# mhozza/covest

Hardware: NVIDIA B200
Metric: loglik_point_bin_evals_per_sec (higher is better)
Workload: dtype f64

## Files before the change

### covest_b200/csrc/capi.cu

```cuda
#include <cuda_runtime.h>

#include <cmath>
#include <cstdio>
#include <cstdlib>
#include <algorithm>
#include <cstring>
#include <string>
#include <utility>
#include <vector>

#include "../../include/covest_b200.h"
#include "cvtables.h"
#include "factored.h"
#include "faithful.h"
#include "kernels.h"
#include "kmers.h"

#define CVB_CHUNK_POINTS (1LL << 22)
#define CVB_MAX_TIMED_CHUNKS 64
#define CVB_TOPK_RADIX_MIN 32768

struct cvb_ctx {
    int device = 0;
    int n_sm = 0;
// ... 277 lines not shown
            const char *rows = getenv("COVEST_B200_ROWS");
            const bool compact = !(rows && !strcmp(rows, "full"));
            CvHostTables RT;
            const bool row_tables = compact && tail == 0.0 && cv_build_row_tables(T, bin_j, bin_h, RT);
            c->fdesc = m;
            if (row_tables) {
                CvModelDesc &f = c->fdesc;
                f.n_groups = RT.n_groups;
                f.na = RT.na;
                f.n_blocks = RT.n_blocks;
                f.tab.slot_mult = f.tab.slot_h = nullptr;
                f.tab.slot_bin = nullptr;
                if ((e = upload_profile_tables(c, RT, f.tab)) != cudaSuccess) break;
            }
            const CvHostTables &FT = row_tables ? RT : T;
            std::vector<int> line_map;
            std::vector<double2> mh;
            std::vector<double> row_h;
            cvf_build_slots(FT.slot_mult, FT.slot_h, compact, row_tables, line_map, mh, row_h, &c->slots.sum_line);
            c->slots.nsteps = (int)(row_h.size() / 64);
            if ((e = upload(c, line_map, &c->slots.line_map)) != cudaSuccess) break;
            if ((e = upload(c, mh, &c->slots.slot_mh)) != cudaSuccess) break;
            if ((e = upload(c, cvf_step_masks(row_h), &c->slots.step_mask)) != cudaSuccess) break;
            c->slots.counts_first = cvf_counts_first(row_h);
            std::vector<double> lt(2 * CV_LOG_N);
            cv_log_table(lt.data());
            if ((e = upload(c, lt, &c->d_log_tab)) != cudaSuccess) break;
        }
        if (const char *pm = getenv("COVEST_B200_PATH"))
            c->path_mode = !strcmp(pm, "direct") ? 1 : !strcmp(pm, "factored") ? 2 : !strcmp(pm, "gemm") ? 3
                           : !strcmp(pm, "prefix") ? 4 : !strcmp(pm, "faithful") ? 5 : 0;
        if (const char *wl = getenv("COVEST_B200_PROFILE_MIB"))
            if (atoll(wl) > 0)
                c->w_limit = (size_t)atoll(wl) * (1 << 20) / sizeof(double);
        if (const char *po = getenv("COVEST_B200_POISON")) {
            c->poison = !strcmp(po, "nan") ? 0xFF : !strcmp(po, "finite") ? 0x7F : 0;
            if (!c->poison && *po) {
                rc = fail(nullptr, CVB_EINVAL, "COVEST_B200_POISON must be nan or finite");
                break;
// ... 645 lines not shown

extern "C" int cvb_last_path_info(cvb_ctx *ctx, double *out, int n_out)
{
    if (!ctx || !out || n_out < 1)
        return CVB_EINVAL;
    CU(cudaSetDevice(ctx->device), "cudaSetDevice");
    double v[CVB_PATH_INFO_LEN] = {0};
    v[0] = ctx->last_path;
    {
        unsigned long long fixed = 0;
        CU(cudaMemcpy(&fixed, ctx->d_fixed, sizeof(fixed), cudaMemcpyDeviceToHost), "cudaMemcpy");
        v[9] = (double)fixed;
    }
    if (ctx->last_path >= 2) {
        v[10] = (double)ctx->fw.analytic;
        v[11] = (double)(ctx->slots.nsteps * 64 - (ctx->slots.sum_line >= 0 ? 32 : 0));
        const CvFactorWork &w = ctx->fw;
        v[1] = (double)w.n_groups;
        v[2] = (double)w.n_tiles;
        v[3] = (double)w.n_items;
        v[4] = (double)w.w_doubles;
        v[8] = (double)w.n_runs;
        if (w.timed && w.ev[0]) {
            float ms = 0.f;
            CU(cudaEventSynchronize(w.ev[3]), "cudaEventSynchronize");
            CU(cudaEventElapsedTime(&ms, w.ev[0], w.ev[1]), "cudaEventElapsedTime");
            v[5] = ms;
            CU(cudaEventElapsedTime(&ms, w.ev[1], w.ev[2]), "cudaEventElapsedTime");
            v[6] = ms;
            CU(cudaEventElapsedTime(&ms, w.ev[2], w.ev[3]), "cudaEventElapsedTime");
            v[7] = ms;
// ... 330 lines not shown
```

### covest_b200/csrc/factored.cu

```cuda
#include "factored.h"

#include <cub/device/device_radix_sort.cuh>
#include <cub/block/block_scan.cuh>
#include <cub/device/device_scan.cuh>

#include <algorithm>
#include <cstring>
#include <vector>

#include "kdevice.h"

#define CVF_M 128
#define CVF_NS 64
#define CVF_KC 16
#define CVF_THREADS 256
#define CVF_OBITS 20
#define CVF_TILE_DOUBLES (CVF_KC * CVF_NS)

struct CvfPlan {
    unsigned long long *keys, *keys_alt;
    unsigned int *idx, *idx_alt;
    const unsigned int *idx_sorted;
    int *othr;
    int *head, *gid;
// ... 319 lines not shown
{
    int lo = 0, hi = n;
    while (hi - lo > 1) {
        const int step = (hi - lo + 31) >> 5;
        const int p = lo + (lane + 1) * step;
        const bool ok = p < hi && __ldg(start + p) <= x;
        const int cnt = __popc(__ballot_sync(CV_FULL_MASK, ok));
        const int nlo = lo + cnt * step;
        hi = min(nlo + step, hi);
        lo = nlo;
    }
    return lo;
}

#define CVF_STAGE_DOUBLES (CV_GB * CV_NA_MAX * CV_W)

template <int NA>
__device__ __forceinline__ void cvf_store_profile(int lane, int blk, int o, int nsteps,
                                                  const double *__restrict__ slot_mult ,
                                                  const int *__restrict__ line_map, int sum_line, bool sums,
                                                  double *__restrict__ Wg, double *stage, const double *acc)
{
    const int r = lane >> 2, q = lane & 3;
#pragma unroll
    for (int mt = 0; mt < NA; mt++)
#pragma unroll
        for (int c = 0; c < 2; c++) {
            const int chunk = (2 * q + c) ^ (r & 1);
            *reinterpret_cast<double2 *>(stage + (NA * r + mt) * CV_W + 2 * chunk) =
                make_double2(acc[4 * mt + c], acc[4 * mt + 2 + c]);
        }
    __syncwarp();
    double *row0 = Wg + (long long)(o - 1) * nsteps * CVF_NS + lane * 2;
    double2 rest = make_double2(0.0, 0.0);
#pragma unroll
    for (int ns = 0; ns < 2 * NA; ns++) {
        const int row = 4 * ns + (lane >> 3);
        const int chunk = (lane & 7) ^ ((row / NA) & 1);
        double2 v = *reinterpret_cast<const double2 *>(stage + row * CV_W + 2 * chunk);
        const double2 mm = __ldg(reinterpret_cast<const double2 *>(slot_mult) + (blk * (2 * NA) + ns) * 32 + lane);
        v.x = cv_mul(v.x, mm.x);
        v.y = cv_mul(v.y, mm.y);
        const int line = __ldg(line_map + blk * (2 * NA) + ns);
        if (line >= 0) {
            *reinterpret_cast<double2 *>(row0 + line * CVF_NS) = v;
        } else if (sums) {
            rest.x = cv_add(rest.x, v.x);
            rest.y = cv_add(rest.y, v.y);
        }
    }
    if (sum_line >= 0) {
        double *dst = Wg + ((long long)(o - 1) * nsteps + sum_line) * CVF_NS + lane;
        double sum = 0.0;
        if (sums) {
            sum = cv_add(rest.x, rest.y);
            if (blk > 0)
                sum = cv_add(*dst, sum);
        }
        dst[0] = sum;
        dst[32] = 0.0;
    }
    __syncwarp();
}

template <int NA>
__device__ __forceinline__ void cvf_profile_item(int lane, const CvModelDesc &m, CvWarpMem &M,
                                                 int o0, int omax4, int nsteps, const int *__restrict__ line_map,
                                                 int sum_line, double *__restrict__ Wg, double *stage)
{
    const int sp = cvf_copy_slots(m.n_err);
    const int cpt = cvf_copies_per_tile(m.n_err);
    const int kpc = sp >> 2;
    const bool sums = m.tail != 0.0;
    for (int oa = o0; oa < o0 + CVF_KC && oa <= omax4; oa += cpt) {
        cv_w_mass(lane, m, oa, cpt * sp, sp, M);
        __syncwarp();
        const CvTerm tm = cv_w_term(lane, m, oa, cpt * sp, sp, 0, 1.0, M);
        for (int blk = 0; blk < m.n_blocks; blk++) {
            const CvLaneGroup G = cv_lane_group(lane, m, blk, M);
            cv_w_prep<NA>(lane, m, blk, tm, M);
            __syncwarp();
            for (int cc = 0; cc < cpt; cc++) {
                double acc[4 * NA];
#pragma unroll
                for (int i = 0; i < 4 * NA; i++)
                    acc[i] = 0.0;
                cv_w_fused<NA>(lane, G, cc * kpc, (cc + 1) * kpc, *M.fx, acc);
                cvf_store_profile<NA>(lane, blk, oa + cc, nsteps, m.tab.slot_mult_pair, line_map, sum_line, sums, Wg, stage,
                                      acc);
            }
            __syncwarp();
        }
    }
}

__global__ void __launch_bounds__(32 * CV_WARPS_MAX, 1)
cvf_profile_kernel(const __grid_constant__ CvModelDesc m, const __grid_constant__ CvLattice lat,
                   const double *__restrict__ params, int clip, CvfPlan pl, int n_groups,
                   int first_item, int n_items, double *__restrict__ W, long long w_base, int nsteps,
                   const int *__restrict__ line_map, int sum_line, unsigned long long *counter, int groups_staged)
{
    extern __shared__ __align__(16) unsigned char cv_smem_raw[];
    const int lane = threadIdx.x & 31, warp = threadIdx.x >> 5;
    const int S = m.n_err;
    CvWarpMem M;
    {
        double *tab = reinterpret_cast<double *>(cv_smem_raw);
        const int ntab = groups_staged * CV_GD;
        unsigned char *wbase = cv_smem_raw + (size_t)ntab * sizeof(double) + (size_t)warp * cv_warp_bytes(S);
        CvWarpFixed *fx = reinterpret_cast<CvWarpFixed *>(wbase);
        cv_warp_mem_carve(M, fx, reinterpret_cast<double *>(wbase + sizeof(CvWarpFixed)), S);
        for (int i = threadIdx.x; i < ntab; i += blockDim.x)
            tab[i] = m.tab.grp[i];
        M.grp = tab;
    }
// ... 10 lines not shown
            break;
        const int item = first_item + (int)it;
        const int g = cvf_find_warp(pl.item_start, n_groups, item, lane);
        const int kchunk = item - pl.item_start[g];
        const int a = pl.g_start[g];
        const int omax = pl.g_omax[g] - 1;
        const int omax4 = (omax + 3) & ~3;
        double row[CV_MAX_PARAMS];
        cvf_raw_row(m, lat, params, pl.idx_sorted[a], row);
        __syncwarp();
        cv_w_header(lane, m, row, clip, M);
        __syncwarp();
        double *Wg = W + (pl.w_off[g] - w_base);
        const int o0 = kchunk * CVF_KC + 1;
        switch (m.na) {
        case 1: cvf_profile_item<1>(lane, m, M, o0, omax4, nsteps, line_map, sum_line, Wg, stage); break;
        case 2: cvf_profile_item<2>(lane, m, M, o0, omax4, nsteps, line_map, sum_line, Wg, stage); break;
        case 4: cvf_profile_item<4>(lane, m, M, o0, omax4, nsteps, line_map, sum_line, Wg, stage); break;
        default: cvf_profile_item<8>(lane, m, M, o0, omax4, nsteps, line_map, sum_line, Wg, stage); break;
        }
    }
}

#define CVF_STAGES 4
struct CvfSmem {
    double2 Bs[CVF_STAGES][CVF_TILE_DOUBLES / 2];
    double2 As[CVF_STAGES][CVF_M * CVF_KC / 2];
    double red_sum[2][CVF_M];
    double red_mh[2][CVF_M], red_ml[2][CVF_M];
    double log_tab[2 * CV_LOG_N];
    int othr[CVF_M];
    unsigned int pidx[CVF_M];
    int tile;
};
// ... 448 lines not shown

__device__ __forceinline__ int cvf_count_below(const int *a, int n, int x, bool or_equal)
{
    int lo = 0, hi = n;
    while (lo < hi) {
        const int mid = (lo + hi) >> 1;
        const int v = a[mid];
        if (v < x || (or_equal && v == x))
            lo = mid + 1;
        else
            hi = mid;
    }
    return lo;
}

template <bool MASS, bool FULL, bool ONE, int NW, int SL>
__global__ void __launch_bounds__(32 * NW, CVF_WARPS_SM / NW)
cvf_prefix_kernel(const __grid_constant__ CvModelDesc m, const __grid_constant__ CvLattice lat,
                  const double *__restrict__ params, int clip, CvfPlan pl, int first_tile, int n_tiles,
                  const double *__restrict__ W, long long w_base, const double2 *__restrict__ slot_mh,
                  const double *__restrict__ log_tab, int nsteps, int nslots, double *__restrict__ out_ll,
                  unsigned long long *counter, double *__restrict__ scratch)
{
    constexpr int PT_ = 32 * NW, PW_ = NW;
    constexpr int PASS_ = PT_ * SL;
    constexpr int RING_ = CVF_PD * SL * PT_ * 8;
    constexpr int TBUF_ = PW_ * CVF_PE * CVF_PEW;
    extern __shared__ __align__(16) unsigned char cvf_smem_raw[];
    CvfPrefixSmem &S = *reinterpret_cast<CvfPrefixSmem *>(cvf_smem_raw);
    const int tid = threadIdx.x, lane = tid & 31, warp = tid >> 5;
    double *ring = reinterpret_cast<double *>(cvf_smem_raw + CVF_SMEM_HEAD) + tid;
    double *tbuf = reinterpret_cast<double *>(cvf_smem_raw + CVF_SMEM_HEAD + RING_) +
// ... 87 lines not shown
                S.ev[rank] = e;
            }
            if (tid < 2) {
                CvfEvent e;
                e.q1 = e.two = e.many = 0.0;
                e.info = e.need = 0;
                S.ev[npts + tid] = e;
            }
            __syncthreads();

            for (int pass0 = 0; pass0 < nslots; pass0 += PASS_) {
                const int u0 = (pass0 >> 5) + warp;
                const double *src0 = Wg + u0 * 32 + lane;
                constexpr long long SRC_STEP = (long long)PW_ * 32;
                double hcnt[SL];
                int log_mask = 0;
                bool live[SL];
#pragma unroll
                for (int i = 0; i < SL; i++) {
                    const int u = u0 + i * PW_;
                    live[i] = FULL || u * 32 < nslots;
                    const int e = (u & 1) * 32 + lane, L = e >> 1;
                    const int slot = (u >> 1) * CVF_NS + 16 * (L >> 3) + (L & 7) + 8 * (e & 1);
                    hcnt[i] = live[i] ? __ldg(&slot_mh[slot].y) : 0.0;
                    log_mask |= (__any_sync(CV_FULL_MASK, hcnt[i] != 0.0) ? 1 : 0) << i;
                }
                const bool wide = !ONE && log_mask == (1 << SL) - 1;
                auto pair_fast = [&](const double *pa, const double *pb) {
                    unsigned int worst = 0;
#pragma unroll
                    for (int i = 0; i < SL; i++) {
                        const unsigned int ca = (unsigned int)(__double2hiint(pa[i]) - CVF_FAST_LO),
                                           cb = (unsigned int)(__double2hiint(pb[i]) - CVF_FAST_LO);
                        if (hcnt[i] != 0.0)
                            worst = max(worst, max(ca, cb));
                    }
                    return worst < CVF_FAST_SPAN;
                };
                int o_req = 1;
                unsigned int dst_req = ring_s;
                const double *src_req = src0;
                const double *src_far = src0 + (long long)CVF_PL2 * row_stride;
// ... 176 lines not shown
                            const double2 qt = cvf_lds128(ev_a);
                            q1 = qt.x;
                            two = qt.y;
                            cvf_lds_event(ev_a, many, info, need);
                        }
                        k++;
                        double ma = 0.0, mb = 0.0, mla = 0.0, mlb = 0.0;
                        if (MASS) {
#pragma unroll
                            for (int i = 0; i < SL; i++) {
                                cvf_two_sum_acc(ma, mla, pa[i]);
                                cvf_two_sum_acc(mb, mlb, pb[i]);
                            }
                        }
                        double sa = 0.0, sb = 0.0;
                        if (ONE ? log_mask != 0 : log_mask == 1) {
                            const unsigned int ca = (unsigned int)(__double2hiint(pa[0]) - CVF_FAST_LO),
                                               cb = (unsigned int)(__double2hiint(pb[0]) - CVF_FAST_LO);
                            double la, lb;
                            if (ca < CVF_FAST_SPAN && cb < CVF_FAST_SPAN) {
                                la = cvf_log_fast(pa[0], log_s);
                                lb = cvf_log_fast(pb[0], log_s);
                            } else {
                                la = cvf_safe_log(pa[0], log_s);
                                lb = cvf_safe_log(pb[0], log_s);
                            }
                            sa = cv_mul(hcnt[0], la);
                            sb = cv_mul(hcnt[0], lb);
                            if (hcnt[0] == 0.0)
                                sa = sb = 0.0;
                        } else if (wide && pair_fast(pa, pb)) {
#pragma unroll
                            for (int i = 0; i < SL; i++) {
                                const double la = cvf_log_fast(pa[i], log_s),
                                             lb = cvf_log_fast(pb[i], log_s);
                                double ta = cv_mul(hcnt[i], la), tb = cv_mul(hcnt[i], lb);
                                if (hcnt[i] == 0.0)
                                    ta = tb = 0.0;
                                sa = cv_add(sa, ta);
                                sb = cv_add(sb, tb);
                            }
                        } else if (!ONE && log_mask) {
#pragma unroll
                            for (int i = 0; i < SL; i++)
                                if ((log_mask >> i) & 1) {
                                    const unsigned int ca = (unsigned int)(__double2hiint(pa[i]) - CVF_FAST_LO),
                                                       cb = (unsigned int)(__double2hiint(pb[i]) - CVF_FAST_LO);
                                    double la, lb;
                                    if (ca < CVF_FAST_SPAN && cb < CVF_FAST_SPAN) {
                                        la = cvf_log_fast(pa[i], log_s);
                                        lb = cvf_log_fast(pb[i], log_s);
                                    } else {
                                        la = cvf_safe_log(pa[i], log_s);
                                        lb = cvf_safe_log(pb[i], log_s);
                                    }
                                    double ta = cv_mul(hcnt[i], la), tb = cv_mul(hcnt[i], lb);
                                    if (hcnt[i] == 0.0)
                                        ta = tb = 0.0;
                                    sa = cv_add(sa, ta);
                                    sb = cv_add(sb, tb);
                                }
                        }
                        if (pending == CVF_PE - 1) {
                            flush();
                            tb_a = tbuf_s;
                        }
                        cvf_sts64(tb_a, sa);
                        cvf_sts64(tb_a + CVF_PEW * 8, sb);
                        if (MASS) {
                            cvf_sts64(tb_a + TBUF_ * 8, ma);
                            cvf_sts64(tb_a + CVF_PEW * 8 + TBUF_ * 8, mb);
                            cvf_sts64(tb_a + 2 * TBUF_ * 8, mla);
                            cvf_sts64(tb_a + CVF_PEW * 8 + 2 * TBUF_ * 8, mlb);
                        }
                        tb_a += 2 * CVF_PEW * 8;
                        if (lane == pending)
// ... 22 lines not shown
                        CVF_CASE(2)
                        CVF_CASE(3)
#undef CVF_CASE
                    }
                    q1 = qt_next.x;
                    two = qt_next.y;
                    many = many_next;
                    info = info_next;
                    need = need_next;
                    double sum = 0.0, mh = 0.0, ml = 0.0;
                    if (MASS) {
#pragma unroll
                        for (int i = 0; i < SL; i++)
                            cvf_two_sum_acc(mh, ml, p[i]);
                    }
                    if (ONE ? log_mask != 0 : log_mask == 1) {
                        double term = cv_mul(hcnt[0], cvf_safe_log(p[0], log_s));
                        if (hcnt[0] == 0.0)
                            term = 0.0;
                        sum = term;
                    } else if (!ONE && log_mask) {
#pragma unroll
                        for (int i = 0; i < SL; i++)
                            if ((log_mask >> i) & 1) {
                                double term = cv_mul(hcnt[i], cvf_safe_log(p[i], log_s));
                                if (hcnt[i] == 0.0)
                                    term = 0.0;
                                sum = cv_add(sum, term);
                            }
                    }
                    cvf_sts64(tb_a, sum);
                    if (MASS) {
                        cvf_sts64(tb_a + TBUF_ * 8, mh);
                        cvf_sts64(tb_a + 2 * TBUF_ * 8, ml);
                    }
                    tb_a += CVF_PEW * 8;
                    if (lane == pending)
                        mypt = pt;
                    if (++pending == CVF_PE) {
                        flush();
                        tb_a = tbuf_s;
                    }
                }
                if (pending)
// ... 453 lines not shown
    double *A = wk.W + w_need;
    if (wk.poison) {
        CVF_CK(cudaMemsetAsync(wk.W, wk.poison, (w_need + a_need) * sizeof(double), stream));
        CVF_CK(cudaMemsetAsync(wk.d_scratch, wk.poison, (size_t)n_sm * 32 * 3 * CVF_PB * sizeof(double), stream));
    }

    const size_t wb = cv_warp_bytes(m.n_err);
    const int groups_staged = m.n_blocks * CV_GB;
    const size_t tab = (size_t)groups_staged * CV_GD * sizeof(double);
    const size_t wb1 = wb + CVF_STAGE_DOUBLES * sizeof(double);
    int k1_warps = (int)std::min<long long>(CV_WARPS_MAX, ((long long)smem_max - (long long)tab) / (long long)wb1);
    if (k1_warps < 1)
        return cudaErrorInvalidConfiguration;
    const size_t k1_smem = tab + (size_t)k1_warps * wb1;
    const bool want_mass = m.tail != 0.0;
    const int kp_slots = slots_padded - (sl.sum_line >= 0 ? (want_mass || nsteps == 1 ? 32 : CVF_NS) : 0);
    const int kp_half = kp_slots / 32;
    int kp_nw = 8, kp_sl = 4;
    if (kp_half <= 24) {
        static const int nws[] = {1, 2, 3, 4, 6, 8};
        int n3 = 8, n4 = 8;
        for (int i = 5; i >= 0; i--) {
            if (nws[i] * 3 >= kp_half && nws[i] != 4 && nws[i] != 8)
                n3 = nws[i];
            if (nws[i] * 4 >= kp_half)
                n4 = nws[i];
        }
        if (n3 <= n4) {
            kp_nw = n3;
            kp_sl = 3;
        } else {
            kp_nw = n4;
        }
    }
    const size_t kp_smem = cvf_prefix_smem_bytes(want_mass, kp_nw, kp_sl);
    const bool full_passes = kp_slots % (8 * 32 * 4) == 0;
    const bool counts_first = sl.counts_first;
    typedef decltype(&cvf_prefix_kernel<true, true, true, 8, 4>) CvfPrefixFn;
    CvfPrefixFn kp = nullptr;
    const bool full_one = kp_slots == kp_nw * 32 * kp_sl;
#define CVF_PICK(nw_, sl_)                                                                                          \
    (full_one ? (want_mass ? cvf_prefix_kernel<true, true, false, nw_, sl_> : cvf_prefix_kernel<false, true, false, nw_, sl_>) \
              : (want_mass ? cvf_prefix_kernel<true, false, false, nw_, sl_> : cvf_prefix_kernel<false, false, false, nw_, sl_>))
    switch (kp_nw * 10 + kp_sl) {
    case 13: kp = CVF_PICK(1, 3); break;
    case 14: kp = CVF_PICK(1, 4); break;
    case 23: kp = CVF_PICK(2, 3); break;
    case 24: kp = CVF_PICK(2, 4); break;
    case 33: kp = CVF_PICK(3, 3); break;
    case 34: kp = CVF_PICK(3, 4); break;
    case 44: kp = CVF_PICK(4, 4); break;
    case 63: kp = CVF_PICK(6, 3); break;
    case 64: kp = CVF_PICK(6, 4); break;
    default:
        kp = want_mass ? (full_passes ? (counts_first ? cvf_prefix_kernel<true, true, true, 8, 4> : cvf_prefix_kernel<true, true, false, 8, 4>)
                                      : (counts_first ? cvf_prefix_kernel<true, false, true, 8, 4> : cvf_prefix_kernel<true, false, false, 8, 4>))
                       : (full_passes ? (counts_first ? cvf_prefix_kernel<false, true, true, 8, 4> : cvf_prefix_kernel<false, true, false, 8, 4>)
                                      : (counts_first ? cvf_prefix_kernel<false, false, true, 8, 4> : cvf_prefix_kernel<false, false, false, 8, 4>));
    }
#undef CVF_PICK
    CVF_CK(cudaFuncSetAttribute(cvf_profile_kernel, cudaFuncAttributeMaxDynamicSharedMemorySize, (int)k1_smem));
    CVF_CK(cudaFuncSetAttribute(cvf_gemm_kernel, cudaFuncAttributeMaxDynamicSharedMemorySize,
                                (int)sizeof(CvfSmem)));
    CVF_CK(cudaFuncSetAttribute(kp, cudaFuncAttributeMaxDynamicSharedMemorySize, (int)kp_smem));
    if (wk.timed)
        CVF_CK(cudaEventRecord(wk.ev[1], stream));
    for (size_t i = 0; i + 1 < cut.size(); i++) {
        const int g0 = cut[i], g1 = cut[i + 1];
        const int item0 = ranged ? h_item[g0] : 0, item1 = ranged ? h_item[g1] : (int)n_items;
        const int tile0 = ranged ? h_tile[g0] : 0, tile1 = ranged ? h_tile[g1] : (int)n_tiles;
        const long long w0 = ranged ? h_woff[g0] : 0;
        const long long a0 = ranged ? h_achunk[g0] : 0;
        CVF_CK(cudaMemsetAsync(wk.d_counters, 0, 2 * sizeof(unsigned long long), stream));
        if (item1 > item0) {
            const int items = item1 - item0;
            int grid = (items + k1_warps - 1) / k1_warps;
            if (grid > n_sm)
                grid = n_sm;
            cvf_profile_kernel<<<grid, 32 * k1_warps, k1_smem, stream>>>(
                m, lat, params, clip, pl, (int)n_groups, item0, items, wk.W, w0, nsteps, sl.line_map, sl.sum_line,
                wk.d_counters, groups_staged);
            CVF_CK(cudaGetLastError());
            wk.launches++;
        }
        if (tile1 > tile0) {
            const int tiles = tile1 - tile0;
            if (!prefix) {
                cvf_weights_kernel<<<tiles, CVF_THREADS, 0, stream>>>(m, lat, params, clip, pl, tile0, tiles, A, a0);
                CVF_CK(cudaGetLastError());
                wk.launches++;
            }
            if (analytic) {
                cvf_lattice_order<<<(unsigned int)((tiles + tb - 1) / tb), tb, 0, stream>>>(
                    TD, g0, g1, (int)(n_tiles / n_groups), pl.t_order_alt + tile0);
                CVF_CK(cudaGetLastError());
                pl.t_sorted = pl.t_order_alt + tile0;
            } else {
                cub::DoubleBuffer<int> dk(pl.t_key + tile0, pl.t_key_alt + tile0);
                cub::DoubleBuffer<int> dv(pl.t_order + tile0, pl.t_order_alt + tile0);
                size_t tb_ = tmp_bytes;
                CVF_CK(cub::DeviceRadixSort::SortPairsDescending(tmp, tb_, dk, dv, tiles, 0, 32, stream));
                pl.t_sorted = dv.Current();
            }
            if (wk.timed && i + 2 == cut.size())
                CVF_CK(cudaEventRecord(wk.ev[2], stream));
            int grid = tiles < 2 * n_sm ? tiles : 2 * n_sm;
            if (prefix) {
                const int per_sm = std::max(1, std::min(CVF_WARPS_SM / kp_nw, (int)((size_t)smem_max / (kp_smem + 1024))));
                grid = tiles < per_sm * n_sm ? tiles : per_sm * n_sm;
                kp<<<grid, 32 * kp_nw, kp_smem, stream>>>(m, lat, params, clip, pl, tile0, tiles, wk.W, w0, slot_mh,
                                                           log_tab, nsteps, kp_slots, out_ll, wk.d_counters + 1,
                                                           wk.d_scratch);
            } else {
                cvf_gemm_kernel<<<grid, CVF_THREADS, sizeof(CvfSmem), stream>>>(
                    m, pl, tile0, tiles, wk.W, w0, A, a0, slot_mh, step_mask, log_tab, nsteps, out_ll,
                    wk.d_counters + 1);
            }
            CVF_CK(cudaGetLastError());
            wk.launches += 2;
        }
    }
    if (wk.timed)
        CVF_CK(cudaEventRecord(wk.ev[3], stream));
// ... 4 lines not shown
```

### covest_b200/csrc/factored.h

```cpp
#pragma once
#include <cuda_runtime.h>
#include <stdint.h>

#include <vector>

#include "kernels.h"

struct CvfLatticeCache {
    std::vector<double> key;
    std::vector<int> host;
    int M = 0, R = 0, nq = 0, nT = 0, omax = 0;
    int *dev = nullptr;
    size_t dev_cap = 0;
    int *pinned = nullptr;
    size_t pinned_cap = 0;
    cudaEvent_t uploaded = nullptr;
};

struct CvFactorWork {
    void *plan = nullptr;
    size_t plan_cap = 0;
    double *W = nullptr;
    size_t w_cap = 0;
    long long *h_header = nullptr;
// ... 1 lines not shown
    unsigned long long *d_counters = nullptr;
    double *d_scratch = nullptr;
    cudaEvent_t ev[4] = {nullptr, nullptr, nullptr, nullptr};
    bool timed = false;
    long long n_groups = 0, n_tiles = 0, n_items = 0, w_doubles = 0, n_runs = 0;
    int prefix = 0;
    int launches = 0;
    int analytic = 0;
    int poison = 0;
    CvfLatticeCache lattice;
    double gemm_fma = 0.0;
};

struct CvfSlots {
    int nsteps = 0;
    int sum_line = -1;
    const int *line_map = nullptr;
    const double2 *slot_mh = nullptr;
    const int *step_mask = nullptr;
    bool counts_first = false;
};

static inline void cvf_build_slots(const std::vector<double> &slot_mult, const std::vector<double> &slot_h,
                                   bool compact, bool sums, std::vector<int> &line_map, std::vector<double2> &mh,
                                   std::vector<double> &row_h, int *sum_line)
{
    const size_t lines = slot_h.size() / 64;
    line_map.assign(lines, -1);
    mh.clear();
    row_h.clear();
    int kept = 0;
    for (size_t l = 0; l < lines; l++) {
        bool counts = !compact;
        for (int i = 0; i < 64 && !counts; i++)
            counts = slot_h[l * 64 + i] != 0.0;
        if (!counts)
            continue;
        line_map[l] = kept++;
        for (int i = 0; i < 64; i++) {
            double2 v;
            v.x = slot_mult[l * 64 + i];
            v.y = slot_h[l * 64 + i];
            mh.push_back(v);
            row_h.push_back(v.y);
        }
    }
    *sum_line = -1;
    if ((size_t)kept < lines || sums) {
        *sum_line = kept;
        for (int i = 0; i < 64; i++) {
            double2 v;
            v.x = 1.0;
            v.y = 0.0;
            mh.push_back(v);
            row_h.push_back(0.0);
        }
    }
}

bool cvf_supported(const CvModelDesc &m);

cudaError_t cvf_eval(const CvModelDesc &m, const CvLattice &lat, const double *const *lat_axes_host,
                     const double *params, long long n,
                     int clip, double *out_ll, const CvfSlots &sl,
                     const double *log_tab, CvFactorWork &wk, int n_sm, int smem_max, size_t w_limit,
                     double min_group, double min_run, int kernel_mode, cudaStream_t stream,
                     int *used);

static inline std::vector<int> cvf_step_masks(const std::vector<double> &slot_h)
{
    std::vector<int> out(slot_h.size() / 32, 0);
    for (size_t s = 0; s < slot_h.size(); s++)
        if (slot_h[s] != 0.0) {
            const int in32 = (int)(s & 31), nt = in32 >> 3, c = in32 & 1;
            out[s / 32] |= 1 << (2 * nt + c);
        }
    return out;
}

static inline bool cvf_counts_first(const std::vector<double> &slot_h)
{
    for (size_t s = 0; s < slot_h.size(); s++)
        if (slot_h[s] != 0.0 && (((2 * (s / 64) + (s % 64) / 32) % 32) >> 3) != 0)
            return false;
    return true;
}

void cvf_release(CvFactorWork &wk);
```

### covest_b200/engine.py

```python
import ctypes
import math
import os

import numpy as np

from . import _capi


class DeviceError(RuntimeError):
    """An error reported by libcovest_b200 (bad argument or CUDA failure)."""


def default_device():
    for var in ('COVEST_B200_DEVICE', 'LOCAL_RANK'):
        v = os.environ.get(var)
        if v not in (None, ''):
            return int(v)
    return 0


def _is_torch_cuda(x):
    return hasattr(x, 'data_ptr') and hasattr(x, 'is_cuda') and x.is_cuda


# ... 216 lines not shown
                    'cvb_last_kernel_ms')
        return ms.value, n.value

    def last_launches(self):
        n = ctypes.c_int()
        self._check(self._lib.cvb_last_kernel_ms(self._ctx, None, ctypes.byref(n)), 'cvb_last_kernel_ms')
        return n.value

    PATH_AUTO, PATH_PER_POINT, PATH_FACTORED, PATH_FACTORED_GEMM, PATH_FACTORED_PREFIX = 0, 1, 2, 3, 4
    PATH_TERM_BY_TERM = 5

    def set_path(self, mode):
        self._check(self._lib.cvb_set_path(self._ctx, int(mode)), 'cvb_set_path')

    def last_path_info(self):
        buf = (ctypes.c_double * 12)()
        self._check(self._lib.cvb_last_path_info(self._ctx, buf, 12), 'cvb_last_path_info')
        v = list(buf)
        return {'path': {1: 'per-point', 2: 'factored', 3: 'factored', 4: 'term-by-term'}.get(int(v[0]), 'none'),
                'kernel': {1: 'cv_loglik_kernel', 2: 'cvf_gemm_kernel', 3: 'cvf_prefix_kernel',
                           4: 'cv_faithful_kernel'}.get(int(v[0]), 'none'),
                'groups': int(v[1]), 'tiles': int(v[2]), 'items': int(v[3]), 'profile_doubles': int(v[4]),
                'plan_ms': v[5], 'profile_ms': v[6], 'gemm_ms': v[7], 'q_runs': int(v[8]),
                'refined_points': int(v[9]), 'analytic_plan': bool(v[10]), 'row_slots': int(v[11])}

    @property
    def sm_count(self):
        return self._lib.cvb_device_sm_count(self._ctx)
```

### include/covest_b200.h

```cpp
#ifndef COVEST_B200_H
#define COVEST_B200_H

#include <stdint.h>

#ifdef __cplusplus
extern "C" {
#endif

#if defined(__GNUC__)
#define CVB_API __attribute__((visibility("default")))
#else
#define CVB_API
#endif

#define CVB_OK 0
#define CVB_EINVAL (-1)
#define CVB_ECUDA (-2)
#define CVB_ENOMEM (-3)

#define CVB_MODEL_BASIC 0
#define CVB_MODEL_REPEATS 1

typedef struct cvb_ctx cvb_ctx;

// ... 23 lines not shown
CVB_API int cvb_lattice_eval(cvb_ctx *ctx, const int32_t *axis_len, const double *axis_values,
                     int64_t first, int64_t stride, int64_t block, int64_t count, double *out_ll,
                     int k_best, double *out_rows, void *stream);

CVB_API int cvb_lattice_profile(cvb_ctx *ctx, const int32_t *axis_len, const double *axis_values,
                                int64_t first, int64_t stride, int64_t block, int64_t count,
                                uint32_t keep_mask, double *out_rows, void *stream);

CVB_API int cvb_fp64_peak(cvb_ctx *ctx, int kind, int reps, double *out_tflops);

CVB_API int cvb_set_timing(cvb_ctx *ctx, int enabled);
CVB_API int cvb_last_kernel_ms(cvb_ctx *ctx, double *out_ms, int *out_launches);

CVB_API int cvb_set_path(cvb_ctx *ctx, int mode);

#define CVB_PATH_INFO_LEN 12
CVB_API int cvb_last_path_info(cvb_ctx *ctx, double *out, int n_out);

CVB_API int cvb_n_param(const cvb_ctx *ctx);
CVB_API int cvb_device_sm_count(const cvb_ctx *ctx);
CVB_API const char *cvb_version(void);

typedef struct cvb_kmer_table cvb_kmer_table;

CVB_API int cvb_kmer_table_create(int k, int64_t capacity, int part, int n_parts, int device,
                                  cvb_kmer_table **out);
CVB_API void cvb_kmer_table_destroy(cvb_kmer_table *t);
CVB_API const char *cvb_kmer_last_error(const cvb_kmer_table *t);

CVB_API int cvb_kmer_clear(cvb_kmer_table *t, void *stream);

// ... 14 lines not shown
```

Baseline: 774.6 billion.

## Pack nonzero-count profile slots densely instead of keeping whole 64-slot lines

The profile layout now keeps only the individual slots with nonzero histogram weight, packed contiguously with a per-slot gather map into the swizzled staging buffer, rather than keeping whole 64-slot lines. The prefix kernel therefore reads and takes logs over fewer profile entries, and the log_mask / counts_first special-case branches are dropped in favour of a uniform loop. The profile store becomes an indexed gather with partial stores. SL>4 variants get a lower occupancy bound. The risks are gather overhead and unaligned scalar stores in the profile kernel.

```diff
diff --git a/covest_b200/csrc/capi.cu b/covest_b200/csrc/capi.cu
--- a/covest_b200/csrc/capi.cu
+++ b/covest_b200/csrc/capi.cu
@@ -315,15 +315,18 @@
                 if ((e = upload_profile_tables(c, RT, f.tab)) != cudaSuccess) break;
             }
             const CvHostTables &FT = row_tables ? RT : T;
-            std::vector<int> line_map;
-            std::vector<double2> mh;
-            std::vector<double> row_h;
-            cvf_build_slots(FT.slot_mult, FT.slot_h, compact, row_tables, line_map, mh, row_h, &c->slots.sum_line);
-            c->slots.nsteps = (int)(row_h.size() / 64);
-            if ((e = upload(c, line_map, &c->slots.line_map)) != cudaSuccess) break;
-            if ((e = upload(c, mh, &c->slots.slot_mh)) != cudaSuccess) break;
-            if ((e = upload(c, cvf_step_masks(row_h), &c->slots.step_mask)) != cudaSuccess) break;
-            c->slots.counts_first = cvf_counts_first(row_h);
+            CvfRowLayout L;
+            cvf_build_slots(FT.slot_mult, FT.slot_h, FT.n_blocks, compact, row_tables, L);
+            c->slots.nsteps = L.nsteps;
+            c->slots.body = L.body;
+            c->slots.sum_half = L.sum_half;
+            c->slots.line_slots = L.line_slots;
+            if ((e = upload(c, L.at, &c->slots.at)) != cudaSuccess) break;
+            if ((e = upload(c, L.mult, &c->slots.mult)) != cudaSuccess) break;
+            if ((e = upload(c, L.blk_first, &c->slots.blk_first)) != cudaSuccess) break;
+            if ((e = upload(c, L.in_row, &c->slots.in_row)) != cudaSuccess) break;
+            if ((e = upload(c, L.mh, &c->slots.slot_mh)) != cudaSuccess) break;
+            if ((e = upload(c, cvf_step_masks(L.row_h), &c->slots.step_mask)) != cudaSuccess) break;
             std::vector<double> lt(2 * CV_LOG_N);
             cv_log_table(lt.data());
             if ((e = upload(c, lt, &c->d_log_tab)) != cudaSuccess) break;
@@ -999,7 +1002,8 @@
     }
     if (ctx->last_path >= 2) {
         v[10] = (double)ctx->fw.analytic;
-        v[11] = (double)(ctx->slots.nsteps * 64 - (ctx->slots.sum_line >= 0 ? 32 : 0));
+        v[11] = (double)ctx->slots.line_slots;
+        v[12] = (double)(ctx->slots.sum_half >= 0 ? 32 * (ctx->slots.sum_half + 1) : 64 * ctx->slots.nsteps);
         const CvFactorWork &w = ctx->fw;
         v[1] = (double)w.n_groups;
         v[2] = (double)w.n_tiles;
diff --git a/covest_b200/csrc/factored.cu b/covest_b200/csrc/factored.cu
--- a/covest_b200/csrc/factored.cu
+++ b/covest_b200/csrc/factored.cu
@@ -357,11 +357,11 @@
 }
 
 #define CVF_STAGE_DOUBLES (CV_GB * CV_NA_MAX * CV_W)
+#define CVF_GATHER 4
 
 template <int NA>
-__device__ __forceinline__ void cvf_store_profile(int lane, int blk, int o, int nsteps,
-                                                  const double *__restrict__ slot_mult ,
-                                                  const int *__restrict__ line_map, int sum_line, bool sums,
+__device__ __forceinline__ void cvf_store_profile(int lane, int blk, int k0, int k1, int o, const CvfSlots &sl,
+                                                  const double *__restrict__ slot_mult , bool sums,
                                                   double *__restrict__ Wg, double *stage, const double *acc)
 {
     const int r = lane >> 2, q = lane & 3;
@@ -369,31 +369,66 @@
     for (int mt = 0; mt < NA; mt++)
 #pragma unroll
         for (int c = 0; c < 2; c++) {
-            const int chunk = (2 * q + c) ^ (r & 1);
+            const int chunk = (2 * q + c) ^ cvf_stage_swizzle(NA * r + mt, NA);
             *reinterpret_cast<double2 *>(stage + (NA * r + mt) * CV_W + 2 * chunk) =
                 make_double2(acc[4 * mt + c], acc[4 * mt + 2 + c]);
         }
     __syncwarp();
-    double *row0 = Wg + (long long)(o - 1) * nsteps * CVF_NS + lane * 2;
+    double *row = Wg + (long long)(o - 1) * sl.nsteps * CVF_NS;
+    const int ka = 16 * (lane >> 3) + (lane & 7);
+    for (int l0 = k0 >> 6; 64 * l0 < k1; l0 += CVF_GATHER) {
+        int2 at[CVF_GATHER];
+        double2 mm[CVF_GATHER];
+#pragma unroll
+        for (int i = 0; i < CVF_GATHER; i++) {
+            const int a = 64 * (l0 + i) + ka, b = a + 8;
+            const bool ia = a >= k0 && a < k1, ib = b >= k0 && b < k1;
+            at[i] = make_int2(-2, -2);
+            mm[i] = make_double2(0.0, 0.0);
+            if (ia || ib) {
+                at[i] = __ldg(sl.at + 32 * (l0 + i) + lane);
+                mm[i] = __ldg(sl.mult + 32 * (l0 + i) + lane);
+                at[i].x = ia ? at[i].x : -2;
+                at[i].y = ib ? at[i].y : -2;
+            }
+        }
+#pragma unroll
+        for (int i = 0; i < CVF_GATHER; i++) {
+            double2 v = make_double2(0.0, 0.0);
+            if (at[i].x >= 0)
+                v.x = cv_mul(stage[at[i].x], mm[i].x);
+            if (at[i].y >= 0)
+                v.y = cv_mul(stage[at[i].y], mm[i].y);
+            double *dst = row + 64 * (l0 + i) + 2 * lane;
+            if (at[i].x >= -1 && at[i].y >= -1) {
+                *reinterpret_cast<double2 *>(dst) = v;
+            } else {
+                if (at[i].x >= -1)
+                    dst[0] = v.x;
+                if (at[i].y >= -1)
+                    dst[1] = v.y;
+            }
+        }
+    }
     double2 rest = make_double2(0.0, 0.0);
-#pragma unroll
-    for (int ns = 0; ns < 2 * NA; ns++) {
-        const int row = 4 * ns + (lane >> 3);
-        const int chunk = (lane & 7) ^ ((row / NA) & 1);
-        double2 v = *reinterpret_cast<const double2 *>(stage + row * CV_W + 2 * chunk);
-        const double2 mm = __ldg(reinterpret_cast<const double2 *>(slot_mult) + (blk * (2 * NA) + ns) * 32 + lane);
-        v.x = cv_mul(v.x, mm.x);
-        v.y = cv_mul(v.y, mm.y);
-        const int line = __ldg(line_map + blk * (2 * NA) + ns);
-        if (line >= 0) {
-            *reinterpret_cast<double2 *>(row0 + line * CVF_NS) = v;
-        } else if (sums) {
-            rest.x = cv_add(rest.x, v.x);
-            rest.y = cv_add(rest.y, v.y);
-        }
-    }
-    if (sum_line >= 0) {
-        double *dst = Wg + ((long long)(o - 1) * nsteps + sum_line) * CVF_NS + lane;
+    if (sums) {
+#pragma unroll
+        for (int ns = 0; ns < 2 * NA; ns++) {
+            const int srow = 4 * ns + (lane >> 3);
+            const int chunk = (lane & 7) ^ cvf_stage_swizzle(srow, NA);
+            double2 v = *reinterpret_cast<const double2 *>(stage + srow * CV_W + 2 * chunk);
+            const double2 mm = __ldg(reinterpret_cast<const double2 *>(slot_mult) + (blk * (2 * NA) + ns) * 32 + lane);
+            v.x = cv_mul(v.x, mm.x);
+            v.y = cv_mul(v.y, mm.y);
+            const unsigned long long in_row = __ldg(sl.in_row + blk * (2 * NA) + ns) >> (16 * (lane >> 3) + (lane & 7));
+            if (!(in_row & 1))
+                rest.x = cv_add(rest.x, v.x);
+            if (!((in_row >> 8) & 1))
+                rest.y = cv_add(rest.y, v.y);
+        }
+    }
+    if (sl.sum_half >= 0) {
+        double *dst = row + 32 * sl.sum_half + lane;
         double sum = 0.0;
         if (sums) {
             sum = cv_add(rest.x, rest.y);
@@ -401,15 +436,16 @@
                 sum = cv_add(*dst, sum);
         }
         dst[0] = sum;
-        dst[32] = 0.0;
+        if (!(sl.sum_half & 1))
+            dst[32] = 0.0;
     }
     __syncwarp();
 }
 
 template <int NA>
 __device__ __forceinline__ void cvf_profile_item(int lane, const CvModelDesc &m, CvWarpMem &M,
-                                                 int o0, int omax4, int nsteps, const int *__restrict__ line_map,
-                                                 int sum_line, double *__restrict__ Wg, double *stage)
+                                                 int o0, int omax4, const CvfSlots &sl, double *__restrict__ Wg,
+                                                 double *stage)
 {
     const int sp = cvf_copy_slots(m.n_err);
     const int cpt = cvf_copies_per_tile(m.n_err);
@@ -420,6 +456,7 @@
         __syncwarp();
         const CvTerm tm = cv_w_term(lane, m, oa, cpt * sp, sp, 0, 1.0, M);
         for (int blk = 0; blk < m.n_blocks; blk++) {
+            const int k0 = __ldg(sl.blk_first + blk), k1 = __ldg(sl.blk_first + blk + 1);
             const CvLaneGroup G = cv_lane_group(lane, m, blk, M);
             cv_w_prep<NA>(lane, m, blk, tm, M);
             __syncwarp();
@@ -429,8 +466,7 @@
                 for (int i = 0; i < 4 * NA; i++)
                     acc[i] = 0.0;
                 cv_w_fused<NA>(lane, G, cc * kpc, (cc + 1) * kpc, *M.fx, acc);
-                cvf_store_profile<NA>(lane, blk, oa + cc, nsteps, m.tab.slot_mult_pair, line_map, sum_line, sums, Wg, stage,
-                                      acc);
+                cvf_store_profile<NA>(lane, blk, k0, k1, oa + cc, sl, m.tab.slot_mult_pair, sums, Wg, stage, acc);
             }
             __syncwarp();
         }
@@ -440,8 +476,8 @@
 __global__ void __launch_bounds__(32 * CV_WARPS_MAX, 1)
 cvf_profile_kernel(const __grid_constant__ CvModelDesc m, const __grid_constant__ CvLattice lat,
                    const double *__restrict__ params, int clip, CvfPlan pl, int n_groups,
-                   int first_item, int n_items, double *__restrict__ W, long long w_base, int nsteps,
-                   const int *__restrict__ line_map, int sum_line, unsigned long long *counter, int groups_staged)
+                   int first_item, int n_items, double *__restrict__ W, long long w_base, CvfSlots sl,
+                   unsigned long long *counter, int groups_staged)
 {
     extern __shared__ __align__(16) unsigned char cv_smem_raw[];
     const int lane = threadIdx.x & 31, warp = threadIdx.x >> 5;
@@ -482,10 +518,10 @@
         double *Wg = W + (pl.w_off[g] - w_base);
         const int o0 = kchunk * CVF_KC + 1;
         switch (m.na) {
-        case 1: cvf_profile_item<1>(lane, m, M, o0, omax4, nsteps, line_map, sum_line, Wg, stage); break;
-        case 2: cvf_profile_item<2>(lane, m, M, o0, omax4, nsteps, line_map, sum_line, Wg, stage); break;
-        case 4: cvf_profile_item<4>(lane, m, M, o0, omax4, nsteps, line_map, sum_line, Wg, stage); break;
-        default: cvf_profile_item<8>(lane, m, M, o0, omax4, nsteps, line_map, sum_line, Wg, stage); break;
+        case 1: cvf_profile_item<1>(lane, m, M, o0, omax4, sl, Wg, stage); break;
+        case 2: cvf_profile_item<2>(lane, m, M, o0, omax4, sl, Wg, stage); break;
+        case 4: cvf_profile_item<4>(lane, m, M, o0, omax4, sl, Wg, stage); break;
+        default: cvf_profile_item<8>(lane, m, M, o0, omax4, sl, Wg, stage); break;
         }
     }
 }
@@ -964,8 +1000,8 @@
     return lo;
 }
 
-template <bool MASS, bool FULL, bool ONE, int NW, int SL>
-__global__ void __launch_bounds__(32 * NW, CVF_WARPS_SM / NW)
+template <bool MASS, bool FULL, int NW, int SL>
+__global__ void __launch_bounds__(32 * NW, (SL > 4 ? CVF_WARPS_SM / 2 : CVF_WARPS_SM) / NW)
 cvf_prefix_kernel(const __grid_constant__ CvModelDesc m, const __grid_constant__ CvLattice lat,
                   const double *__restrict__ params, int clip, CvfPlan pl, int first_tile, int n_tiles,
                   const double *__restrict__ W, long long w_base, const double2 *__restrict__ slot_mh,
@@ -1083,18 +1119,13 @@
                 const double *src0 = Wg + u0 * 32 + lane;
                 constexpr long long SRC_STEP = (long long)PW_ * 32;
                 double hcnt[SL];
-                int log_mask = 0;
                 bool live[SL];
 #pragma unroll
                 for (int i = 0; i < SL; i++) {
                     const int u = u0 + i * PW_;
                     live[i] = FULL || u * 32 < nslots;
-                    const int e = (u & 1) * 32 + lane, L = e >> 1;
-                    const int slot = (u >> 1) * CVF_NS + 16 * (L >> 3) + (L & 7) + 8 * (e & 1);
-                    hcnt[i] = live[i] ? __ldg(&slot_mh[slot].y) : 0.0;
-                    log_mask |= (__any_sync(CV_FULL_MASK, hcnt[i] != 0.0) ? 1 : 0) << i;
+                    hcnt[i] = live[i] ? __ldg(&slot_mh[32 * u + cvf_half_slot(lane)].y) : 0.0;
                 }
-                const bool wide = !ONE && log_mask == (1 << SL) - 1;
                 auto pair_fast = [&](const double *pa, const double *pb) {
                     unsigned int worst = 0;
 #pragma unroll
@@ -1301,22 +1332,7 @@
                             }
                         }
                         double sa = 0.0, sb = 0.0;
-                        if (ONE ? log_mask != 0 : log_mask == 1) {
-                            const unsigned int ca = (unsigned int)(__double2hiint(pa[0]) - CVF_FAST_LO),
-                                               cb = (unsigned int)(__double2hiint(pb[0]) - CVF_FAST_LO);
-                            double la, lb;
-                            if (ca < CVF_FAST_SPAN && cb < CVF_FAST_SPAN) {
-                                la = cvf_log_fast(pa[0], log_s);
-                                lb = cvf_log_fast(pb[0], log_s);
-                            } else {
-                                la = cvf_safe_log(pa[0], log_s);
-                                lb = cvf_safe_log(pb[0], log_s);
-                            }
-                            sa = cv_mul(hcnt[0], la);
-                            sb = cv_mul(hcnt[0], lb);
-                            if (hcnt[0] == 0.0)
-                                sa = sb = 0.0;
-                        } else if (wide && pair_fast(pa, pb)) {
+                        if (pair_fast(pa, pb)) {
 #pragma unroll
                             for (int i = 0; i < SL; i++) {
                                 const double la = cvf_log_fast(pa[i], log_s),
@@ -1327,26 +1343,16 @@
                                 sa = cv_add(sa, ta);
                                 sb = cv_add(sb, tb);
                             }
-                        } else if (!ONE && log_mask) {
-#pragma unroll
-                            for (int i = 0; i < SL; i++)
-                                if ((log_mask >> i) & 1) {
-                                    const unsigned int ca = (unsigned int)(__double2hiint(pa[i]) - CVF_FAST_LO),
-                                                       cb = (unsigned int)(__double2hiint(pb[i]) - CVF_FAST_LO);
-                                    double la, lb;
-                                    if (ca < CVF_FAST_SPAN && cb < CVF_FAST_SPAN) {
-                                        la = cvf_log_fast(pa[i], log_s);
-                                        lb = cvf_log_fast(pb[i], log_s);
-                                    } else {
-                                        la = cvf_safe_log(pa[i], log_s);
-                                        lb = cvf_safe_log(pb[i], log_s);
-                                    }
-                                    double ta = cv_mul(hcnt[i], la), tb = cv_mul(hcnt[i], lb);
-                                    if (hcnt[i] == 0.0)
-                                        ta = tb = 0.0;
-                                    sa = cv_add(sa, ta);
-                                    sb = cv_add(sb, tb);
-                                }
+                        } else {
+#pragma unroll
+                            for (int i = 0; i < SL; i++) {
+                                double ta = cv_mul(hcnt[i], cvf_safe_log(pa[i], log_s)),
+                                       tb = cv_mul(hcnt[i], cvf_safe_log(pb[i], log_s));
+                                if (hcnt[i] == 0.0)
+                                    ta = tb = 0.0;
+                                sa = cv_add(sa, ta);
+                                sb = cv_add(sb, tb);
+                            }
                         }
                         if (pending == CVF_PE - 1) {
                             flush();
@@ -1399,20 +1405,12 @@
                         for (int i = 0; i < SL; i++)
                             cvf_two_sum_acc(mh, ml, p[i]);
                     }
-                    if (ONE ? log_mask != 0 : log_mask == 1) {
-                        double term = cv_mul(hcnt[0], cvf_safe_log(p[0], log_s));
-                        if (hcnt[0] == 0.0)
+#pragma unroll
+                    for (int i = 0; i < SL; i++) {
+                        double term = cv_mul(hcnt[i], cvf_safe_log(p[i], log_s));
+                        if (hcnt[i] == 0.0)
                             term = 0.0;
-                        sum = term;
-                    } else if (!ONE && log_mask) {
-#pragma unroll
-                        for (int i = 0; i < SL; i++)
-                            if ((log_mask >> i) & 1) {
-                                double term = cv_mul(hcnt[i], cvf_safe_log(p[i], log_s));
-                                if (hcnt[i] == 0.0)
-                                    term = 0.0;
-                                sum = cv_add(sum, term);
-                            }
+                        sum = cv_add(sum, term);
                     }
                     cvf_sts64(tb_a, sum);
                     if (MASS) {
@@ -1896,10 +1894,13 @@
         return cudaErrorInvalidConfiguration;
     const size_t k1_smem = tab + (size_t)k1_warps * wb1;
     const bool want_mass = m.tail != 0.0;
-    const int kp_slots = slots_padded - (sl.sum_line >= 0 ? (want_mass || nsteps == 1 ? 32 : CVF_NS) : 0);
+    const int kp_slots = sl.sum_half < 0 ? slots_padded : 32 * (want_mass || sl.body == 0 ? sl.body + 1 : sl.body);
     const int kp_half = kp_slots / 32;
     int kp_nw = 8, kp_sl = 4;
-    if (kp_half <= 24) {
+    if (kp_half >= 5 && kp_half <= 7) {
+        kp_nw = 1;
+        kp_sl = 7;
+    } else if (kp_half <= 24) {
         static const int nws[] = {1, 2, 3, 4, 6, 8};
         int n3 = 8, n4 = 8;
         for (int i = 5; i >= 0; i--) {
@@ -1916,17 +1917,16 @@
         }
     }
     const size_t kp_smem = cvf_prefix_smem_bytes(want_mass, kp_nw, kp_sl);
-    const bool full_passes = kp_slots % (8 * 32 * 4) == 0;
-    const bool counts_first = sl.counts_first;
-    typedef decltype(&cvf_prefix_kernel<true, true, true, 8, 4>) CvfPrefixFn;
+    typedef decltype(&cvf_prefix_kernel<true, true, 8, 4>) CvfPrefixFn;
     CvfPrefixFn kp = nullptr;
-    const bool full_one = kp_slots == kp_nw * 32 * kp_sl;
+    const bool full = kp_slots % (kp_nw * 32 * kp_sl) == 0;
 #define CVF_PICK(nw_, sl_)                                                                                          \
-    (full_one ? (want_mass ? cvf_prefix_kernel<true, true, false, nw_, sl_> : cvf_prefix_kernel<false, true, false, nw_, sl_>) \
-              : (want_mass ? cvf_prefix_kernel<true, false, false, nw_, sl_> : cvf_prefix_kernel<false, false, false, nw_, sl_>))
+    (full ? (want_mass ? cvf_prefix_kernel<true, true, nw_, sl_> : cvf_prefix_kernel<false, true, nw_, sl_>) \
+          : (want_mass ? cvf_prefix_kernel<true, false, nw_, sl_> : cvf_prefix_kernel<false, false, nw_, sl_>))
     switch (kp_nw * 10 + kp_sl) {
     case 13: kp = CVF_PICK(1, 3); break;
     case 14: kp = CVF_PICK(1, 4); break;
+    case 17: kp = CVF_PICK(1, 7); break;
     case 23: kp = CVF_PICK(2, 3); break;
     case 24: kp = CVF_PICK(2, 4); break;
     case 33: kp = CVF_PICK(3, 3); break;
@@ -1934,11 +1934,7 @@
     case 44: kp = CVF_PICK(4, 4); break;
     case 63: kp = CVF_PICK(6, 3); break;
     case 64: kp = CVF_PICK(6, 4); break;
-    default:
-        kp = want_mass ? (full_passes ? (counts_first ? cvf_prefix_kernel<true, true, true, 8, 4> : cvf_prefix_kernel<true, true, false, 8, 4>)
-                                      : (counts_first ? cvf_prefix_kernel<true, false, true, 8, 4> : cvf_prefix_kernel<true, false, false, 8, 4>))
-                       : (full_passes ? (counts_first ? cvf_prefix_kernel<false, true, true, 8, 4> : cvf_prefix_kernel<false, true, false, 8, 4>)
-                                      : (counts_first ? cvf_prefix_kernel<false, false, true, 8, 4> : cvf_prefix_kernel<false, false, false, 8, 4>));
+    default: kp = CVF_PICK(8, 4); break;
     }
 #undef CVF_PICK
     CVF_CK(cudaFuncSetAttribute(cvf_profile_kernel, cudaFuncAttributeMaxDynamicSharedMemorySize, (int)k1_smem));
@@ -1960,8 +1956,7 @@
             if (grid > n_sm)
                 grid = n_sm;
             cvf_profile_kernel<<<grid, 32 * k1_warps, k1_smem, stream>>>(
-                m, lat, params, clip, pl, (int)n_groups, item0, items, wk.W, w0, nsteps, sl.line_map, sl.sum_line,
-                wk.d_counters, groups_staged);
+                m, lat, params, clip, pl, (int)n_groups, item0, items, wk.W, w0, sl, wk.d_counters, groups_staged);
             CVF_CK(cudaGetLastError());
             wk.launches++;
         }
@@ -1988,7 +1983,8 @@
                 CVF_CK(cudaEventRecord(wk.ev[2], stream));
             int grid = tiles < 2 * n_sm ? tiles : 2 * n_sm;
             if (prefix) {
-                const int per_sm = std::max(1, std::min(CVF_WARPS_SM / kp_nw, (int)((size_t)smem_max / (kp_smem + 1024))));
+                const int per_sm = std::max(1, std::min((kp_sl > 4 ? CVF_WARPS_SM / 2 : CVF_WARPS_SM) / kp_nw,
+                                                        (int)((size_t)smem_max / (kp_smem + 1024))));
                 grid = tiles < per_sm * n_sm ? tiles : per_sm * n_sm;
                 kp<<<grid, 32 * kp_nw, kp_smem, stream>>>(m, lat, params, clip, pl, tile0, tiles, wk.W, w0, slot_mh,
                                                            log_tab, nsteps, kp_slots, out_ll, wk.d_counters + 1,
diff --git a/covest_b200/csrc/factored.h b/covest_b200/csrc/factored.h
--- a/covest_b200/csrc/factored.h
+++ b/covest_b200/csrc/factored.h
@@ -39,48 +39,95 @@
 
 struct CvfSlots {
     int nsteps = 0;
-    int sum_line = -1;
-    const int *line_map = nullptr;
+    int body = 0;
+    int sum_half = -1;
+    int line_slots = 0;
+    const int2 *at = nullptr;
+    const double2 *mult = nullptr;
+    const int *blk_first = nullptr;
+    const unsigned long long *in_row = nullptr;
     const double2 *slot_mh = nullptr;
     const int *step_mask = nullptr;
-    bool counts_first = false;
+};
+
+#ifdef __CUDACC__
+__host__ __device__
+#endif
+static inline int cvf_half_slot(int lane)
+{
+    return 16 * (lane >> 4) + ((lane >> 1) & 7) + 8 * (lane & 1);
+}
+
+#ifdef __CUDACC__
+__host__ __device__
+#endif
+static inline int cvf_stage_swizzle(int srow, int na)
+{
+    return ((srow / na) & 1) ^ ((srow & 3) << 1);
+}
+
+struct CvfRowLayout {
+    std::vector<int> src, blk_first;
+    std::vector<unsigned long long> in_row;
+    std::vector<int2> at;
+    std::vector<double2> mh, mult;
+    std::vector<double> row_h;
+    int nsteps = 0, body = 0, sum_half = -1, line_slots = 0;
 };
 
 static inline void cvf_build_slots(const std::vector<double> &slot_mult, const std::vector<double> &slot_h,
-                                   bool compact, bool sums, std::vector<int> &line_map, std::vector<double2> &mh,
-                                   std::vector<double> &row_h, int *sum_line)
+                                   int n_blocks, bool pack, bool row_tables, CvfRowLayout &L)
 {
-    const size_t lines = slot_h.size() / 64;
-    line_map.assign(lines, -1);
-    mh.clear();
-    row_h.clear();
-    int kept = 0;
-    for (size_t l = 0; l < lines; l++) {
-        bool counts = !compact;
-        for (int i = 0; i < 64 && !counts; i++)
-            counts = slot_h[l * 64 + i] != 0.0;
-        if (!counts)
-            continue;
-        line_map[l] = kept++;
-        for (int i = 0; i < 64; i++) {
-            double2 v;
-            v.x = slot_mult[l * 64 + i];
-            v.y = slot_h[l * 64 + i];
-            mh.push_back(v);
-            row_h.push_back(v.y);
+    const size_t n = slot_h.size(), per_blk = n / n_blocks;
+    L.src.clear();
+    L.blk_first.assign(n_blocks + 1, 0);
+    L.in_row.assign(n / 64, 0ULL);
+    size_t lines_counted = 0;
+    for (size_t l = 0; l < n / 64; l++) {
+        bool counts = false;
+        for (int i = 0; i < 64; i++)
+            counts = counts || slot_h[l * 64 + i] != 0.0;
+        lines_counted += counts;
+    }
+    for (size_t t = 0; t < n; t++) {
+        if (t % per_blk == 0)
+            L.blk_first[t / per_blk] = (int)L.src.size();
+        if (!pack || slot_h[t] != 0.0) {
+            L.in_row[t / 64] |= 1ULL << (t % 64);
+            L.src.push_back((int)t);
         }
     }
-    *sum_line = -1;
-    if ((size_t)kept < lines || sums) {
-        *sum_line = kept;
-        for (int i = 0; i < 64; i++) {
-            double2 v;
-            v.x = 1.0;
-            v.y = 0.0;
-            mh.push_back(v);
-            row_h.push_back(0.0);
+    L.body = (int)(L.src.size() + 31) / 32;
+    L.blk_first[n_blocks] = 32 * L.body;
+    L.sum_half = pack ? L.body : -1;
+    L.nsteps = pack ? (L.body + 2) / 2 : L.body / 2;
+    L.src.resize((size_t)64 * L.nsteps, -1);
+    L.mh.assign(L.src.size(), double2{0.0, 0.0});
+    L.row_h.assign(L.src.size(), 0.0);
+    for (size_t k = 0; k < L.src.size(); k++)
+        if (L.src[k] >= 0) {
+            L.mh[k] = double2{slot_mult[L.src[k]], slot_h[L.src[k]]};
+            L.row_h[k] = slot_h[L.src[k]];
         }
+    const int na = (int)(per_blk / (CV_GB * CV_W));
+    auto stage_at = [&](int t) {
+        if (t < 0)
+            return -1;
+        t = (int)(t % per_blk);
+        const int srow = t >> 4, col = t & 15;
+        return srow * CV_W + 2 * ((col & 7) ^ cvf_stage_swizzle(srow, na)) + (col >> 3);
+    };
+    L.at.resize(L.src.size() / 2);
+    L.mult.resize(L.src.size() / 2);
+    for (size_t i = 0; i < L.at.size(); i++) {
+        const size_t a = 64 * (i / 32) + 16 * ((i % 32) >> 3) + (i & 7), b = a + 8;
+        L.at[i] = int2{stage_at(L.src[a]), stage_at(L.src[b])};
+        L.mult[i] = double2{L.mh[a].x, L.mh[b].x};
     }
+    if (pack)
+        for (int i = 0; i < 32; i++)
+            L.mh[32 * L.sum_half + i].x = 1.0;
+    L.line_slots = !pack ? (int)n : (int)(64 * lines_counted) + (lines_counted < n / 64 || row_tables ? 32 : 0);
 }
 
 bool cvf_supported(const CvModelDesc &m);
@@ -103,12 +150,4 @@
     return out;
 }
 
-static inline bool cvf_counts_first(const std::vector<double> &slot_h)
-{
-    for (size_t s = 0; s < slot_h.size(); s++)
-        if (slot_h[s] != 0.0 && (((2 * (s / 64) + (s % 64) / 32) % 32) >> 3) != 0)
-            return false;
-    return true;
-}
-
 void cvf_release(CvFactorWork &wk);
diff --git a/covest_b200/engine.py b/covest_b200/engine.py
--- a/covest_b200/engine.py
+++ b/covest_b200/engine.py
@@ -254,15 +254,16 @@
         self._check(self._lib.cvb_set_path(self._ctx, int(mode)), 'cvb_set_path')
 
     def last_path_info(self):
-        buf = (ctypes.c_double * 12)()
-        self._check(self._lib.cvb_last_path_info(self._ctx, buf, 12), 'cvb_last_path_info')
+        buf = (ctypes.c_double * 13)()
+        self._check(self._lib.cvb_last_path_info(self._ctx, buf, 13), 'cvb_last_path_info')
         v = list(buf)
         return {'path': {1: 'per-point', 2: 'factored', 3: 'factored', 4: 'term-by-term'}.get(int(v[0]), 'none'),
                 'kernel': {1: 'cv_loglik_kernel', 2: 'cvf_gemm_kernel', 3: 'cvf_prefix_kernel',
                            4: 'cv_faithful_kernel'}.get(int(v[0]), 'none'),
                 'groups': int(v[1]), 'tiles': int(v[2]), 'items': int(v[3]), 'profile_doubles': int(v[4]),
                 'plan_ms': v[5], 'profile_ms': v[6], 'gemm_ms': v[7], 'q_runs': int(v[8]),
-                'refined_points': int(v[9]), 'analytic_plan': bool(v[10]), 'row_slots': int(v[11])}
+                'refined_points': int(v[9]), 'analytic_plan': bool(v[10]), 'row_slots': int(v[11]),
+                'packed_slots': int(v[12])}
 
     @property
     def sm_count(self):
diff --git a/include/covest_b200.h b/include/covest_b200.h
--- a/include/covest_b200.h
+++ b/include/covest_b200.h
@@ -61,7 +61,7 @@
 
 CVB_API int cvb_set_path(cvb_ctx *ctx, int mode);
 
-#define CVB_PATH_INFO_LEN 12
+#define CVB_PATH_INFO_LEN 13
 CVB_API int cvb_last_path_info(cvb_ctx *ctx, double *out, int n_out);
 
 CVB_API int cvb_n_param(const cvb_ctx *ctx);
```

Result: faster. 808.9 billion, median of 6 (+4.4%).
